# johncreed/one-class-ffm

Hardware: AMD Instinct MI355X
Metric: train instances/sec, kkbox-shape k=32; 1/2/4/8 MI355X vs CPU OpenMP (higher is better)
Workload: dtype f32; 1 GPU; kkbox-shape (BASELINE configs[2]): one-class FFM block Newton-CG epoch; rows_per_gpu=30755, rows_total=30755, items=100000, positives=2127663, user_fields=2, item_fields=3, k=32, parallelism=dp1, rccl_ranks=0, launcher=none, allreduce=none

## Files before the change

### one-class-ffm_amd/csrc/kernels.hpp

```cpp
#pragma once

#include <hip/hip_runtime.h>
#include <stdint.h>

#include <type_traits>

namespace ocffm {

typedef float f4v __attribute__((ext_vector_type(4)));
typedef double d2v __attribute__((ext_vector_type(2)));
typedef double d4v __attribute__((ext_vector_type(4)));

#ifndef OCFFM_F64_WIDE
#define OCFFM_F64_WIDE 1
#endif
template <typename real> struct VT;
template <> struct VT<float> {
  using V = f4v;
  static constexpr int N = 4;
};
template <> struct VT<double> {
  using V = std::conditional_t<OCFFM_F64_WIDE != 0, d4v, d2v>;
  static constexpr int N = OCFFM_F64_WIDE ? 4 : 2;
};
// ... 2572 lines not shown
                                                      const real *__restrict__ src, real *__restrict__ dst,
                                                      const int *__restrict__ skip) {
  if (skip && *skip) return;
  for (uint64_t q = ((uint64_t)blockIdx.x * BLOCK + threadIdx.x) * 4; q < n; q += (uint64_t)gridDim.x * BLOCK * 4) {
    if (q + 4 <= n) {
      const uint4 ix = *reinterpret_cast<const uint4 *>(idx + q);
      const real a = src[ix.x], b = src[ix.y], c = src[ix.z], d = src[ix.w];
      dst[q] = a;
      dst[q + 1] = b;
      dst[q + 2] = c;
      dst[q + 3] = d;
    } else {
      for (uint64_t r = q; r < n; r++) dst[r] = src[idx[r]];
    }
  }
}

template <typename real, int KP>
__global__ __launch_bounds__(BLOCK) void k_update_side_row(uint64_t R, const int64_t *__restrict__ xptr,
                                                           const uint32_t *__restrict__ xidx,
                                                           const real *__restrict__ xval, const real *__restrict__ S,
                                                           real *__restrict__ P1, const real *__restrict__ Q1,
                                                           real *__restrict__ a1, bool one, real *__restrict__ W,
                                                           const real *__restrict__ Pd, const CgState *st,
                                                           double *__restrict__ asum, double *part, unsigned *tick,
                                                           const int *__restrict__ skip, uint64_t nfold) {
  using G = Geo<real, KP>;
  if (skip && *skip) return;
  WAVE_SETUP
  const int sg = lane / G::LPR, li = lane % G::LPR;
  const real alpha = ((W || nfold) && st->nr_cg >= 1) ? (real)st->alpha : (real)0;
  double bs = 0;
  for (uint64_t i = wave * G::NSG + sg; i < R; i += nwaves * G::NSG) {
    vec_t<real> xs = vzero<real>();
    if (nfold) {
      for (int64_t p = one ? (int64_t)i : xptr[i]; p < (one ? (int64_t)i + 1 : xptr[i + 1]); p++)
        xs += vsplat<real>(xval[p]) * final_step<real>(S, Pd, alpha, (size_t)xidx[p] * KP + li * G::VE);
    } else if (W) {
      xs = vsplat<real>(xval[i]) * apply_owned_row<real, KP>(S, Pd, W, alpha, (size_t)xidx[i] * KP + li * G::VE);
    } else if (one) {
      xs = vsplat<real>(xval[i]) * vld<real>(S + (size_t)xidx[i] * KP + li * G::VE);
    } else {
      for (int64_t p = xptr[i]; p < xptr[i + 1]; p++)
        xs += vsplat<real>(xval[p]) * vld<real>(S + (size_t)xidx[p] * KP + li * G::VE);
    }
    vst<real>(P1 + i * KP + li * G::VE, vld<real>(P1 + i * KP + li * G::VE) + xs);
    const real gap = sg_sum<G::LPR>(hsum<real>(xs * vld<real>(Q1 + i * KP + li * G::VE)));
    if (li == 0) {
      const real an = a1[i] + gap;
      a1[i] = an;
      bs += (double)an;
    }
  }
  if (nfold) fold_apply<real>(nfold, S, Pd, W, alpha);
  const double bv[1] = {block_sum(bs)};
  double tot[1];
  if (last_block<1>(bv, part, tick, tot) && threadIdx.x == 0) asum[0] = tot[0];
}

template <typename real, int KP, int SPT>
__global__ __launch_bounds__(BLOCK) void k_gram_part(uint64_t Rp, int L, const real *const *__restrict__ A,
                                                     const real *__restrict__ B, const real *__restrict__ wv,
                                                     double *__restrict__ part, uint64_t rows_per_block,
                                                     int sub_per_y) {
  constexpr int Q4 = KP / 4;
  constexpr int TR = (KP >= 64) ? 16 : 32;
  constexpr int VE = VT<real>::N;
  extern __shared__ __align__(16) unsigned char smem_raw[];
  real *sA = reinterpret_cast<real *>(smem_raw);
  real *sB = sA + (size_t)L * TR * KP;
  real *sW = sB + (size_t)TR * KP;
  const int t = threadIdx.x;
  const int nsub_tot = L * Q4 * Q4;
  const int sub0 = blockIdx.y * sub_per_y;
  const int nsub = max(0, min(sub_per_y, nsub_tot - sub0));
  real acc[SPT][16];
#pragma unroll
  for (int q = 0; q < SPT; q++)
#pragma unroll
    for (int x = 0; x < 16; x++) acc[q][x] = 0;
  real cs = 0, ws = 0, wtot = 0;
  const uint64_t r0 = (uint64_t)blockIdx.x * rows_per_block;
  const uint64_t r1 = min(Rp, r0 + rows_per_block);
  const bool do_cols = blockIdx.y == 0;
  const int pieces_row = KP / VE;
  const int ntab = L + (B ? 1 : 0);
  for (uint64_t j0 = r0; j0 < r1; j0 += TR) {
    const int nr = (int)min<uint64_t>(TR, r1 - j0);
    __syncthreads();
    const int tot = ntab * TR * pieces_row;
    for (int q = t; q < tot; q += BLOCK) {
      const int tab = q / (TR * pieces_row);
      const int rr = (q / pieces_row) % TR;
      const int pc = q % pieces_row;
      vec_t<real> v = vzero<real>();
      if (rr < nr) v = vld<real>((tab < L ? A[tab] : B) + (j0 + rr) * KP + pc * VE);
      vst<real>((tab < L ? sA + ((size_t)tab * TR + rr) * KP : sB + (size_t)rr * KP) + pc * VE, v);
    }
    if (wv && t < TR) sW[t] = t < nr ? wv[j0 + t] : (real)0;
    __syncthreads();
#pragma unroll
    for (int q = 0; q < SPT; q++) {
      if (t + q * BLOCK < nsub) {
        const int sub = sub0 + t + q * BLOCK;
        const int l = sub / (Q4 * Q4), eq = (sub / Q4) % Q4, dq = sub % Q4;
        const real *pa = sA + (size_t)l * TR * KP + eq * 4;
        const real *pb = sB + dq * 4;
        for (int rr = 0; rr < nr; rr++) {
          real av[4], bv[4];
#pragma unroll
          for (int x = 0; x < 4; x++) {
            av[x] = pa[rr * KP + x];
            bv[x] = pb[rr * KP + x];
          }
#pragma unroll
          for (int x = 0; x < 4; x++)
#pragma unroll
            for (int y = 0; y < 4; y++) acc[q][x * 4 + y] += av[x] * bv[y];
        }
      }
    }
    if (do_cols && t < KP && B) {
      for (int rr = 0; rr < nr; rr++) {
        const real bb = sB[rr * KP + t];
        cs += bb;
        if (wv) ws += sW[rr] * bb;
      }
    }
    if (do_cols && t == 0 && wv)
      for (int rr = 0; rr < nr; rr++) wtot += sW[rr];
  }
  const size_t NOUT = (size_t)L * KP * KP + 2 * KP + 1;
  double *out = part + (size_t)blockIdx.x * NOUT;
#pragma unroll
  for (int q = 0; q < SPT; q++) {
    if (t + q * BLOCK < nsub) {
      const int sub = sub0 + t + q * BLOCK;
      const int l = sub / (Q4 * Q4), eq = (sub / Q4) % Q4, dq = sub % Q4;
#pragma unroll
      for (int x = 0; x < 4; x++)
#pragma unroll
        for (int y = 0; y < 4; y++) out[((size_t)l * KP + eq * 4 + x) * KP + dq * 4 + y] = (double)acc[q][x * 4 + y];
    }
  }
  if (do_cols) {
    if (t < KP) {
      out[(size_t)L * KP * KP + t] = (double)cs;
      out[(size_t)L * KP * KP + KP + t] = (double)ws;
    }
    if (t == 0) out[(size_t)L * KP * KP + 2 * KP] = (double)wtot;
  }
}

template <int L>
__global__ __launch_bounds__(BLOCK) void k_gram_mfma32(uint64_t Rp, const float *const *__restrict__ A,
                                                      const float *__restrict__ B, const float *__restrict__ wv,
                                                      float *__restrict__ part, uint64_t rows_per_block) {
  typedef float f16x __attribute__((ext_vector_type(16)));
  constexpr int U = 4;
  __shared__ float red[L][1024];
  __shared__ float redc[3][32];
  const int lane = threadIdx.x & 63, w = threadIdx.x >> 6;
  const int e = lane & 31, hf = lane >> 5;
  f16x acc[L];
#pragma unroll
  for (int c = 0; c < L; c++)
#pragma unroll
    for (int r = 0; r < 16; r++) acc[c][r] = 0.0f;
  BufView ab[L];
#pragma unroll
  for (int c = 0; c < L; c++) ab[c] = buf_view(A[c], Rp * 128);
  const BufView bb = buf_view(B, B ? Rp * 128 : 0), wb = buf_view(wv, wv ? Rp * 4 : 0);
  float cs = 0, ws = 0, wt = 0;
  const uint64_t r0 = (uint64_t)blockIdx.x * rows_per_block;
  const uint64_t r1 = min(Rp, r0 + rows_per_block);
  float bv[2][U], wvv[2][U], av[2][U][L];
  auto load = [&](int sb, uint64_t j0) {
#pragma unroll
    for (int u = 0; u < U; u++) {
      const uint64_t jj = j0 + 8 * u + hf;
      const bool ok = jj < r1;
      const uint32_t off = ok ? (uint32_t)(jj * 128 + e * 4) : 0xffffffffu;
      bv[sb][u] = bld1<float>(bb, off);
      wvv[sb][u] = bld1<float>(wb, ok ? (uint32_t)(jj * 4) : 0xffffffffu);
#pragma unroll
      for (int c = 0; c < L; c++) av[sb][u][c] = bld1<float>(ab[c], off);
    }
  };
  auto step = [&](int sb) {
#pragma unroll
    for (int u = 0; u < U; u++) {
#pragma unroll
      for (int c = 0; c < L; c++) acc[c] = __builtin_amdgcn_mfma_f32_32x32x2f32(av[sb][u][c], bv[sb][u], acc[c], 0, 0, 0);
      cs += bv[sb][u];
      ws += wvv[sb][u] * bv[sb][u];
      if (e == 0) wt += wvv[sb][u];
    }
  };
  for (uint64_t j0 = r0 + 2 * w; j0 < r1; j0 += 16 * U) {
    load(0, j0);
    load(1, j0 + 8 * U);
    step(0);
    step(1);
  }
  cs += __shfl_xor(cs, 32, 64);
  ws += __shfl_xor(ws, 32, 64);
  wt += __shfl_xor(wt, 32, 64);
  for (int ww = 0; ww < BLOCK / 64; ww++) {
    if (w == ww) {
#pragma unroll
      for (int c = 0; c < L; c++)
#pragma unroll
          for (int r = 0; r < 16; r++) {
            const int m = 8 * (r >> 2) + 4 * hf + (r & 3);
            float &x = red[c][m * 32 + e];
            x = (ww == 0 ? 0.0f : x) + acc[c][r];
          }
      if (hf == 0) {
        redc[0][e] = (ww == 0 ? 0.0f : redc[0][e]) + cs;
        redc[1][e] = (ww == 0 ? 0.0f : redc[1][e]) + ws;
        if (e == 0) redc[2][0] = (ww == 0 ? 0.0f : redc[2][0]) + wt;
      }
    }
    __syncthreads();
  }
  const size_t NOUT = (size_t)L * 1024 + 2 * 32 + 1;
  float *out = part + (size_t)blockIdx.x * NOUT;
  for (int o = threadIdx.x; o < L * 1024; o += BLOCK) out[o] = red[o >> 10][o & 1023];
  if (threadIdx.x < 32) {
    out[(size_t)L * 1024 + threadIdx.x] = redc[0][threadIdx.x];
    out[(size_t)L * 1024 + 32 + threadIdx.x] = redc[1][threadIdx.x];
  }
  if (threadIdx.x == 0) out[(size_t)L * 1024 + 64] = redc[2][0];
}

constexpr int GW64 = 1;
static __global__ __launch_bounds__(BLOCK, 3) void k_gram_mfma64(uint64_t Rp, int C, const float *const *__restrict__ A,
                                                       const float *__restrict__ B, const float *__restrict__ wv,
                                                       float *__restrict__ part, uint64_t nout,
                                                       uint64_t rows_per_block, unsigned ngroups, unsigned nwork) {
  typedef float f16x __attribute__((ext_vector_type(16)));
  constexpr int U = 4;
  const int lane = threadIdx.x & 63, w = threadIdx.x >> 6;
  const int e = lane & 31, hf = lane >> 5;
  const unsigned L = (gridDim.x & 7u) ? blockIdx.x : xcd_work_item(blockIdx.x, gridDim.x);
  if (L >= nwork) return;
  const unsigned grp = L % ngroups, chunk = L / ngroups;
  const int c0 = (int)(grp * (BLOCK / 64) + w);
  if (c0 > C) return;
  f16x acc[4];
#pragma unroll
  for (int t = 0; t < 4; t++)
#pragma unroll
    for (int r = 0; r < 16; r++) acc[t][r] = 0.0f;
  const BufView bb = buf_view(B, Rp * 256);
  const uint64_t r0 = (uint64_t)chunk * rows_per_block;
  const uint64_t r1 = r0 + rows_per_block < Rp ? r0 + rows_per_block : Rp;
  float *out = part + (size_t)chunk * nout;
  if (c0 == C) {
    const BufView wb = buf_view(wv, wv ? Rp * 4 : 0);
    float wt = 0;
    for (uint64_t j0 = r0; j0 < r1; j0 += 2 * U) {
      float bv[U][2], sv[U];
#pragma unroll
      for (int u = 0; u < U; u++) {
        const uint64_t jj = j0 + 2 * u + hf;
        const bool ok = jj < r1;
        const uint32_t off = ok ? (uint32_t)(jj * 256 + e * 4) : 0xffffff00u;
#pragma unroll
        for (int h = 0; h < 2; h++) bv[u][h] = bld1<float>(bb, off + h * 128);
        const float wvi = bld1<float>(wb, ok ? (uint32_t)(jj * 4) : 0xffffff00u);
        sv[u] = e == 0 ? 1.0f : (e == 1 ? wvi : 0.0f);
        if (e == 0) wt += wvi;
      }
#pragma unroll
      for (int u = 0; u < U; u++)
#pragma unroll
        for (int nt = 0; nt < 2; nt++) acc[nt] = __builtin_amdgcn_mfma_f32_32x32x2f32(sv[u], bv[u][nt], acc[nt], 0, 0, 0);
    }
    wt += __shfl_xor(wt, 32, 64);
    if (hf == 0) {
#pragma unroll
      for (int nt = 0; nt < 2; nt++) {
        out[(size_t)C * 4096 + nt * 32 + e] = acc[nt][0];
        out[(size_t)C * 4096 + 64 + nt * 32 + e] = acc[nt][1];
      }
      if (e == 0) out[(size_t)C * 4096 + 128] = wt;
    }
    return;
  }
  const BufView ab = buf_view(A[c0], Rp * 256);
  float bv[2][U][2], av[2][U][2];
  auto load = [&](int sb, uint64_t j0) {
#pragma unroll
    for (int u = 0; u < U; u++) {
      const uint64_t jj = j0 + 2 * u + hf;
      const uint32_t off = jj < r1 ? (uint32_t)(jj * 256 + e * 4) : 0xffffff00u;
#pragma unroll
      for (int h = 0; h < 2; h++) {
        bv[sb][u][h] = bld1<float>(bb, off + h * 128);
        av[sb][u][h] = bld1<float>(ab, off + h * 128);
      }
    }
  };
  auto step = [&](int sb) {
#pragma unroll
    for (int u = 0; u < U; u++)
#pragma unroll
      for (int mt = 0; mt < 2; mt++)
#pragma unroll
        for (int nt = 0; nt < 2; nt++)
          acc[mt * 2 + nt] = __builtin_amdgcn_mfma_f32_32x32x2f32(av[sb][u][mt], bv[sb][u][nt], acc[mt * 2 + nt], 0, 0, 0);
  };
  for (uint64_t j0 = r0; j0 < r1; j0 += 4 * U) {
    load(0, j0);
    load(1, j0 + 2 * U);
    step(0);
    step(1);
  }
#pragma unroll
  for (int t = 0; t < 4; t++)
#pragma unroll
    for (int r = 0; r < 16; r++) {
      const int m = (t >> 1) * 32 + 8 * (r >> 2) + 4 * hf + (r & 3), n = (t & 1) * 32 + e;
      out[(size_t)c0 * 4096 + m * 64 + n] = acc[t][r];
    }
}

static __global__ __launch_bounds__(BLOCK) void k_gram_mfma_f64(uint64_t Rp, int C, const double *const *__restrict__ A,
                                                               const double *__restrict__ B,
                                                               const double *__restrict__ wv, double *__restrict__ part,
                                                               uint64_t nout, uint64_t rows_per_block,
                                                               unsigned ngroups, unsigned nwork) {
  typedef double d4 __attribute__((ext_vector_type(4)));
  constexpr int U = 4;
  const int lane = threadIdx.x & 63, w = threadIdx.x >> 6;
  const int c16 = lane & 15, rq = lane >> 4;
  const unsigned L = (gridDim.x & 7u) ? blockIdx.x : xcd_work_item(blockIdx.x, gridDim.x);
  if (L >= nwork) return;
  const unsigned grp = L % ngroups, chunk = L / ngroups;
  const int c0 = (int)(grp * (BLOCK / 64) + w);
  if (c0 > C) return;
  const uint64_t r0 = (uint64_t)chunk * rows_per_block;
  const uint64_t r1 = r0 + rows_per_block < Rp ? r0 + rows_per_block : Rp;
  double *out = part + (size_t)chunk * nout;
  const BufView bb = buf_view(B, Rp * 256);
  if (c0 == C) {
    const BufView wb = buf_view(wv, wv ? Rp * 8 : 0);
    double cs[2] = {0, 0}, ws[2] = {0, 0}, wt = 0;
    for (uint64_t j0 = r0; j0 < r1; j0 += 4 * U) {
#pragma unroll
      for (int u = 0; u < U; u++) {
        const uint64_t jj = j0 + 4 * u + rq;
        const bool ok = jj < r1;
        const uint32_t off = ok ? (uint32_t)(jj * 256 + c16 * 8) : 0xffffff00u;
        const double wvi = bld1<double>(wb, ok ? (uint32_t)(jj * 8) : 0xffffff00u);
#pragma unroll
        for (int h = 0; h < 2; h++) {
          const double b = bld1<double>(bb, off + h * 128);
          cs[h] += b;
          ws[h] += wvi * b;
// ... 276 lines not shown
```

### one-class-ffm_amd/csrc/solver.hip

```cpp
#include <hip/hip_runtime.h>
#include <hip/hip_ext.h>
#include <rccl/rccl.h>

#include <algorithm>
#include <atomic>
#include <charconv>
#include <chrono>
#include <cmath>
#include <cstdio>
#include <cstdlib>
#include <cstring>
#include <fstream>
#include <iomanip>
#include <iostream>
#include <map>
#include <memory>
#include <stdexcept>
#include <string>
#include <thread>
#include <tuple>
#include <unordered_map>
#include <type_traits>
#include <vector>

// ... 1704 lines not shown
    }
    pending_.clear();
  }

  void utx(DevSide<real> &s, uint32_t fi, const real *A, real *out) {
    if (s.R == 0) return;
    DevField<real> &F = *s.F[fi];
    with_kp(kp_, [&](auto K) {
      constexpr int KP = decltype(K)::value;
      using Gm = Geo<real, KP>;
      prof_launch("utx", 0, [&] {
        launch(k_utx<real, KP>, grid_for(s.R, 4 * Gm::NSG), BLOCK, 0, s.R, F.xptr.p, F.xidx.p, F.xval.p, A, out);
      });
    });
  }

  void rowdot_add(uint64_t R, const real *P, const real *Q, real *acc) {
    if (R == 0) return;
    with_kp(kp_, [&](auto K) {
      constexpr int KP = decltype(K)::value;
      using Gm = Geo<real, KP>;
      launch(k_rowdot_add<real, KP>, grid_for(R, 4 * Gm::NSG), BLOCK, 0, R, P, Q, acc);
      HIPCHK(hipGetLastError());
    });
  }

  void bias_sums() {
    for (int sd = 0; sd < 2; sd++) {
      DevSide<real> &s = sd ? V_ : U_;
      launch(k_vec_sum<real>, grid_for(s.R, BLOCK, 256), BLOCK, 0, (uint64_t)s.R, (const real *)s.bias.p,
             bsum_.p + sd, part_.p, tick_.p);
    }
  }

  void calc_side() {
    for (uint32_t f1 = 0; f1 < f_; f1++)
      for (uint32_t f2 = f1; f2 < f_; f2++) {
        if ((f1 < fu_) != (f2 < fu_)) continue;
        const uint32_t b12 = block_index(f1, f2, f_);
        DevSide<real> &s = side(f1);
        rowdot_add(s.R, P_[b12].p, Q_[b12].p, s.bias.p);
      }
  }

  void init_y_tilde() {
    if (U_.R == 0) return;
    with_kp(kp_, [&](auto K) {
      constexpr int KP = decltype(K)::value;
      launch(k_init_ytilde<real, KP>, grid_for(U_.R, 4), BLOCK, 0,
          U_.R, U_.yptr.p, U_.ycol.p, U_.yt.p, V_.yt.p, U_.perm.p, (int)C_, (const real *const *)tabs_.p,
          (const real *const *)(tabs_.p + C_), U_.bias.p, V_.bias.p);
      HIPCHK(hipGetLastError());
    });
  }

  static constexpr int GRAM_LMAX = 8;
  bool mfma_gram(int L) const { return std::is_same<real, float>::value && kp_ == 32 && L >= 1 && !no_mfma_; }

  void aggregates(uint64_t Rp, int L, const real *const *A, const real *B, const real *wv, real *M) {
    const size_t rs = sizeof(real);
    if (mfma_gram64(L, Rp)) {
      gram64(Rp, L, A, B, wv, M);
      return;
    }
    if (std::is_same<real, double>::value && kp_ == 32 && L >= 1 && !no_mfma_ && B_ok(Rp) && M && B) {
      gram_f64(Rp, L, A, B, wv, M);
      return;
    }
    const int TR = kp_ >= 64 ? 16 : 32;
    const bool mg = mfma_gram(L) && (uint64_t)Rp * 128 < 0xffffff00ull;
    const int lmax = mg ? GRAM_LMAX
                                  : std::max<int>(1, (int)((64 * 1024 / rs - (size_t)TR * kp_ - TR) / ((size_t)TR * kp_)));
    int l0 = 0;
    bool first = true;
    do {
      const int Lc = std::min(L - l0, lmax);
      launch_aggr(Rp, Lc, A ? A + l0 : nullptr, B, first ? wv : nullptr, M ? M + (size_t)l0 * kp_ * kp_ : nullptr,
                  first, mg);
      l0 += Lc;
      first = false;
    } while (l0 < L);
  }

  bool mfma_gram64(int L, uint64_t Rp) const {
    return std::is_same<real, float>::value && kp_ == 64 && L >= 1 && !no_mfma_ && B_ok(Rp);
  }
  static bool B_ok(uint64_t Rp) { return Rp * 256 < 0xffffff00ull; }
  void gram64(uint64_t Rp, int L, const real *const *A, const real *B, const real *wv, real *M) {
    if (!M || !B) throw Error(OCFFM_E_STATE, "gram64: Grams and partner table required");
    constexpr int TPB = (BLOCK / 64) * GW64;
    const unsigned gy = (unsigned)((L + 1 + TPB - 1) / TPB);
    const uint64_t nout = (uint64_t)L * 4096 + 129;
    uint64_t nbx = std::max<uint64_t>(1, std::min<uint64_t>((Rp + 63) / 64, std::max<uint64_t>(1, gram64_blocks_ / gy)));
    const uint64_t rpb = ((Rp + nbx - 1) / nbx + 15) / 16 * 16;
    nbx = std::max<uint64_t>(1, (Rp + rpb - 1) / rpb);
    if (gpart64_.n < nbx * nout) gpart64_.alloc(nbx * nout, false);
    const double abytes = (double)Rp * ((L + (B ? 1 : 0)) * 64 + (wv ? 1 : 0)) * sizeof(real);
    const unsigned nwork = (unsigned)(nbx * gy);
    const unsigned grid = xcd_order_ ? (nwork + 7) / 8 * 8 : nwork;
    prof_launch("aggregates", abytes, [&] {
      launch(k_gram_mfma64, grid, BLOCK, 0, Rp, L, (const float *const *)A, (const float *)B,
             (const float *)wv, gpart64_.p, nout, rpb, gy, nwork);
    }, 2.0 * Rp * L * 64 * 64);
    const uint64_t ng = (uint64_t)L * 4096, cnt = ng + 129;
    prof_launch("aggr_reduce", (double)nbx * cnt * 4, [&] {
      launch(k_reduce_parts<real, float>, (unsigned)((cnt + 15) / 16), BLOCK, 0, nbx, nout, (uint64_t)0, cnt,
             (const float *)gpart64_.p, ng, M, sums_.p);
    });
  }

  void gram_f64(uint64_t Rp, int L, const real *const *A, const real *B, const real *wv, real *M) {
    constexpr int TPB = BLOCK / 64;
    const unsigned gy = (unsigned)((L + 1 + TPB - 1) / TPB);
    const uint64_t nout = (uint64_t)L * 1024 + 65;
    uint64_t nbx = std::max<uint64_t>(1, std::min<uint64_t>((Rp + 63) / 64, std::max<uint64_t>(1, gram64_blocks_ / gy)));
    const uint64_t rpb = ((Rp + nbx - 1) / nbx + 31) / 32 * 32;
    nbx = std::max<uint64_t>(1, (Rp + rpb - 1) / rpb);
    if (gpartd_.n < nbx * nout) gpartd_.alloc(nbx * nout, false);
    const double abytes = (double)Rp * ((L + 1) * 32 + (wv ? 1 : 0)) * sizeof(real);
    const unsigned nwork = (unsigned)(nbx * gy);
    const unsigned grid = xcd_order_ ? (nwork + 7) / 8 * 8 : nwork;
    prof_launch("aggregates", abytes, [&] {
      launch(k_gram_mfma_f64, grid, BLOCK, 0, Rp, L, (const double *const *)A, (const double *)B,
             (const double *)wv, gpartd_.p, nout, rpb, gy, nwork);
    }, 2.0 * Rp * L * 32 * 32);
    const uint64_t ng = (uint64_t)L * 1024, cnt = ng + 65;
    prof_launch("aggr_reduce", (double)nbx * cnt * 8, [&] {
      launch(k_reduce_parts<real, double>, (unsigned)((cnt + 15) / 16), BLOCK, 0, nbx, nout, (uint64_t)0, cnt,
             (const double *)gpartd_.p, ng, M, sums_.p);
    });
  }

  void launch_aggr(uint64_t Rp, int L, const real *const *A, const real *B, const real *wv, real *M, bool sums,
                   bool mg) {
    const int TR = kp_ >= 64 ? 16 : 32;
    const size_t smem = ((size_t)L * TR * kp_ + (size_t)TR * kp_ + TR) * sizeof(real);
    const uint64_t nout = (uint64_t)L * kp_ * kp_ + 2 * kp_ + 1;
    const int nsub = L * (kp_ / 4) * (kp_ / 4);
    with_kp(kp_, [&](auto K) {
      constexpr int KP = decltype(K)::value;
      constexpr int SPT = KP >= 64 ? 4 : 2;
      const int sub_per_y = SPT * BLOCK;
      const unsigned gy = (unsigned)std::max(1, (nsub + sub_per_y - 1) / sub_per_y);
      uint64_t nbx = std::max<uint64_t>(1, std::min<uint64_t>((Rp + 63) / 64, 512 / gy));
      nbx = std::min<uint64_t>(nbx, std::max<uint64_t>(1, part_.n / nout));
      const uint64_t rpb = (Rp + nbx - 1) / nbx;
      const double abytes = (double)Rp * ((L + (B ? 1 : 0)) * kp_ + (wv ? 1 : 0)) * sizeof(real);
      if (mg) {
        nbx = std::max<uint64_t>(1, std::min<uint64_t>((Rp + 127) / 128, gram_blocks_));
        nbx = std::min<uint64_t>(nbx, std::max<uint64_t>(1, part_.n / nout));
        const uint64_t rpbm = (Rp + nbx - 1) / nbx;
        prof_launch("aggregates", abytes, [&] {
          auto go = [&](auto lc) {
            launch(k_gram_mfma32<decltype(lc)::value>, (unsigned)nbx, BLOCK, 0, Rp, (const float *const *)A,
                   (const float *)B, (const float *)wv, (float *)part_.p, rpbm);
          };
          switch (L) {
            case 1: go(std::integral_constant<int, 1>()); break;
            case 2: go(std::integral_constant<int, 2>()); break;
            case 3: go(std::integral_constant<int, 3>()); break;
            case 4: go(std::integral_constant<int, 4>()); break;
            case 5: go(std::integral_constant<int, 5>()); break;
            case 6: go(std::integral_constant<int, 6>()); break;
            case 7: go(std::integral_constant<int, 7>()); break;
            default: go(std::integral_constant<int, GRAM_LMAX>()); break;
          }
        });
      } else {
        prof_launch("aggregates", abytes, [&] {
          launch(k_gram_part<real, KP, SPT>, dim3((unsigned)nbx, gy), BLOCK, smem, Rp, L, A, B, wv, part_.p,
                                                                                        rpb, sub_per_y);
        });
      }
      const uint64_t ng = (uint64_t)L * KP * KP;
      const uint64_t gm = M ? ng : 0, off = M ? 0 : ng, cnt = gm + (sums ? 2 * KP + 1 : 0);
      if (cnt)
        prof_launch("aggr_reduce", (double)nbx * cnt * (mg ? 4 : 8), [&] {
          if (mg)
            launch(k_reduce_parts<real, float>, (unsigned)((cnt + 15) / 16), BLOCK, 0, nbx, nout, off, cnt,
                   (const float *)part_.p, gm, M, sums_.p);
          else
            launch(k_reduce_parts<real>, (unsigned)((cnt + 15) / 16), BLOCK, 0, nbx, nout, off, cnt,
                   (const double *)part_.p, gm, M, sums_.p);
        });
      HIPCHK(hipGetLastError());
    });
  }

  void allreduce_dev(real *buf, uint64_t count) {
    if (!comm_.active()) return;
    if (comm_.nccl) {
      NCCLCHK(ncclAllReduce(buf, buf, count, std::is_same<real, double>::value ? ncclDouble : ncclFloat, ncclSum,
                            comm_.nccl, stream_));
    } else {
      HIPCHK(hipMemcpyAsync(stage_, buf, count * sizeof(real), hipMemcpyDeviceToHost, stream_));
      sync();
      if (comm_.host_fn(stage_, count, std::is_same<real, double>::value, comm_.host_user) != 0)
        throw Error(OCFFM_E_COMM, "host all-reduce callback failed");
      HIPCHK(hipMemcpyAsync(buf, stage_, count * sizeof(real), hipMemcpyHostToDevice, stream_));
    }
  }

  void allreduce_dev_d(double *buf, uint64_t count) {
    if (!comm_.active()) return;
    if (comm_.nccl) {
      NCCLCHK(ncclAllReduce(buf, buf, count, ncclDouble, ncclSum, comm_.nccl, stream_));
    } else {
      if (count > DSTAGE) throw Error(OCFFM_E_ARG, "allreduce_dev_d: too many values");
      HIPCHK(hipMemcpyAsync(dstage_, buf, count * sizeof(double), hipMemcpyDeviceToHost, stream_));
      sync();
      if (comm_.host_fn(dstage_, count, 1, comm_.host_user) != 0)
        throw Error(OCFFM_E_COMM, "host all-reduce callback failed");
      HIPCHK(hipMemcpyAsync(buf, dstage_, count * sizeof(double), hipMemcpyHostToDevice, stream_));
    }
  }

  void sync_owned() {
    if (!owned_stale_) return;
    owned_stale_ = false;
    for (uint32_t f1 = 0; f1 < f_; f1++)
      for (uint32_t f2 = f1; f2 < f_; f2++) {
        const uint32_t b12 = block_index(f1, f2, f_);
        if (!blocks_[b12].used) continue;
        for (int t = 0; t < 2; t++) {
          const uint32_t fl = t == 0 ? f1 : f2;
          DevField<real> &F = *side(fl).F[fidx(fl)];
          if (!F.excl) continue;
          real *T = t == 0 ? W_[b12].p : H_[b12].p;
          with_kp(kp_, [&](auto K) {
            constexpr int KP = decltype(K)::value;
            using Gm = Geo<real, KP>;
            const uint64_t nv = F.D * KP / Gm::VE;
            launch(k_mask_rows<real>, grid_for(nv, BLOCK, 2048), BLOCK, 0, nv, T, F.own.p, (uint32_t)Gm::LPR);
          });
          allreduce_dev(T, F.D * kp_);
        }
      }
    sync();
  }

  void allreduce_host(double *buf, uint64_t count) {
    if (!comm_.active()) return;
    if (comm_.nccl) {
      DevBuf<double> d;
      d.upload(buf, count);
      NCCLCHK(ncclAllReduce(d.p, d.p, count, ncclDouble, ncclSum, comm_.nccl, stream_));
      HIPCHK(hipMemcpyAsync(buf, d.p, count * sizeof(double), hipMemcpyDeviceToHost, stream_));
      sync();
    } else if (comm_.host_fn(buf, count, 1, comm_.host_user) != 0) {
      throw Error(OCFFM_E_COMM, "host all-reduce callback failed");
    }
  }

  const double *at_double(DevBuf<real> &at, uint64_t mt) {
    at_d_.alloc(std::max<uint64_t>(mt, 1));
    if (mt) {
      std::vector<real> t(mt);
      HIPCHK(hipMemcpyAsync(t.data(), at.p, mt * sizeof(real), hipMemcpyDeviceToHost, stream_));
      sync();
      std::vector<double> d(t.begin(), t.end());
      HIPCHK(hipMemcpy(at_d_.p, d.data(), mt * sizeof(double), hipMemcpyHostToDevice));
    }
    return at_d_.p;
  }

  struct HalfCtx {
    uint32_t b12, fl, fo;
    bool cross, user;
    DevSide<real> *own, *partner;
    DevField<real> *F;
    uint64_t D;
    real *W1, *P1, *Q1;
    const real *fw;
  };

  HalfCtx half_ctx(uint32_t f1, uint32_t f2, int which) {
    HalfCtx h;
    h.b12 = block_index(f1, f2, f_);
    if (!blocks_[h.b12].used) throw Error(OCFFM_E_ARG, "block not in the model (--ns)");
    h.fl = which == 0 ? f1 : f2;
    h.fo = which == 0 ? f2 : f1;
    h.user = h.fl < fu_;
    h.cross = (f1 < fu_) != (f2 < fu_);
    h.own = &side(h.fl);
    h.partner = h.cross ? &side(h.fo) : h.own;
    h.F = h.own->F[fidx(h.fl)].get();
    h.D = h.F->D;
    h.W1 = which == 0 ? W_[h.b12].p : H_[h.b12].p;
    h.P1 = which == 0 ? P_[h.b12].p : Q_[h.b12].p;
    h.Q1 = which == 0 ? Q_[h.b12].p : P_[h.b12].p;
    h.fw = prm_.freq ? h.F->freqw.p : nullptr;
    return h;
  }

  void gradient(HalfCtx &h) {
    DevSide<real> &own = *h.own;
    if (!(lazy_ok_ && h.cross)) flush_base();
    if (h.cross) ysum_dirty();
    with_kp(kp_, [&](auto K) {
      constexpr int KP = decltype(K)::value;
      using Gm = Geo<real, KP>;
      const double rs = sizeof(real);
      if (h.cross) {
        DevSide<real> &ps = *h.partner;
        aggregates(ps.R, (int)C_, partner_tabs(h), h.Q1, ps.bias.p, M_.p);
        const size_t msz = (size_t)C_ * KP * KP * sizeof(real);
        const bool lds = msz <= 64 * 1024;
        double bytes = (double)own.R * 8 + (double)own.npos * (4 + rs) + (double)ps.R * KP * rs +
// ... 1431 lines not shown
      if (e.tag > nr || (e.tag == -1 && !queued)) e.name += ".noop";
    }
    ccg_now_ = hot_now_ = false;
    cg_log.push_back(nr);
    account_half(h, nr);
    if (hb) {
      hipEvent_t he = ev();
      HIPCHK(hipEventRecord(he, stream_));
      char name[32];
      std::snprintf(name, sizeof(name), "half(%u,%u)%c", f1, f2, which ? 'H' : 'W');
      pending_.push_back({name, 0.0, hb, he, 0, 0.0});
    }
  }

  void finish_half(HalfCtx &h, const int *skip) {
    DevSide<real> &own = *h.own;
    if (h.cross) ysum_dirty();
    else ysum_ok_[h.user ? 1 : 0] = false;
    with_kp(kp_, [&](auto K) {
      constexpr int KP = decltype(K)::value;
      using Gm = Geo<real, KP>;
      const double rs = sizeof(real);
      const uint64_t nv = h.D * KP / Gm::VE;
      const bool excl = h.F->excl;
      if (excl) owned_stale_ = true;
      DevField<real> &F = *h.F;
      const bool fold = F.idlike && own.R > 0 && !excl && !no_fold_;
      const bool rows_kernel = !h.cross || (excl_.on && excl_.b12 == h.b12);
      const bool gfold = !fold && own.R > 0 && !excl && !no_fold_ && gfold_on_ && rows_kernel;
      real *Wf = (fold || gfold) ? h.W1 : nullptr;
      const uint64_t nfold = gfold ? nv : 0;
      const double fbytes = gfold ? (double)h.D * KP * rs * 4 : 0.0;
      if (!fold && !gfold)
        prof_launch("apply_step", (double)h.D * KP * rs * 5, [&] {
          launch(k_apply<real>, grid_for(nv, BLOCK, 2048), BLOCK, 0, nv, Vd_.p, S_.p, h.W1, st_.p,
                 excl ? (const uint8_t *)h.F->own.p : nullptr, (uint32_t)Gm::LPR, skip);
        });
      if (own.R == 0) return;
      if (h.cross) {
        DevSide<real> &other = *h.partner;
        if (excl_.on && excl_.b12 == h.b12) {
          prof_launch("update_cross_rows", (double)own.R * 16 + (double)F.nnz * (4 + rs) + (double)F.D * KP * rs +
                                               (double)own.R * KP * rs * 2 + fbytes, [&] {
            launch(k_update_cross_rows<real, KP>, mfill(k_update_cross_rows<real, KP>, grid_for(own.R, 4 * Gm::NSG)), BLOCK, 0, own.R, F.xptr.p, F.xidx.p,
                   F.xval.p, (const real *)S_.p, h.P1, (real *)nullptr, F.one, Wf, (const real *)Vd_.p,
                   (const CgState *)st_.p, skip, nfold);
          });
          return;
        }
        const double bytes = (double)own.R * 16 + (double)F.nnz * (4 + rs) + (double)F.D * KP * rs +
                             (double)own.R * KP * rs * 2 + (double)own.npos * (4 + 2 * rs) +
                             (double)other.R * KP * rs;
        prof_launch("update_cross_row", bytes, [&] {
          launch(k_update_cross_seg<real, KP>, mfill(k_update_cross_seg<real, KP>, grid_for(own.nseg, 4 * Gm::NSG)), BLOCK, 0,
              own.nseg, own.segs.p, F.xptr.p, F.xidx.p, F.xval.p, S_.p, h.P1, own.ycol.p, own.yt.p, h.Q1,
              (uint64_t)other.R, F.segd.p, F.segx.p, Wf,
              (const real *)Vd_.p, (const CgState *)st_.p, (const real *)nullptr, (const real *)nullptr,
              (const real *)nullptr, skip);
        });
        refresh_other(own, other, skip);
      } else {
        DevSide<real> &other = h.user ? V_ : U_;
        const double bytes = (double)own.R * 16 + (double)F.nnz * (4 + rs) + (double)F.D * KP * rs +
                             (double)own.R * KP * rs * 3 + (double)own.R * rs * 2 + (double)own.npos * (4 + 4 * rs) + fbytes;
        prof_launch("update_side_row", bytes, [&] {
          launch(k_update_side_row<real, KP>, mfill(k_update_side_row<real, KP>, grid_for(own.R, 4 * Gm::NSG)), BLOCK, 0,
              own.R, F.xptr.p, F.xidx.p, F.xval.p, S_.p, h.P1, h.Q1, own.bias.p, F.one, Wf,
              (const real *)Vd_.p, (const CgState *)st_.p, bsum_.p + (h.user ? 0 : 1), part_.p, tick_.p, skip, nfold);
        });
      }
    });
  }

  void account_half(const HalfCtx &h, int c) {
    const double s = sizeof(real), k = (double)kp_;
    const double R = (double)h.own->R, D = (double)h.D, P = (double)h.own->npos;
    const double csr = 8 * R + (double)h.F->nnz * (4 + s);
    if (!h.cross) {
      const double Rp = (double)(h.user ? V_.R : U_.R);
      const double gd = P * s + 8 * R + 2 * R * s + Rp * s + R * k * s + csr + 2 * D * k * s;
      const double hs = c * (8 * R + R * k * s + csr + 9 * D * k * s);
      const double upd = 4 * D * k * s + csr + 3 * R * k * s + 2 * R * s + 2 * P * s + 8 * R;
      alg_bytes += gd + hs + upd;
    } else {
      const double Rp = (double)h.partner->R, Cc = (double)C_;
      const double gd = (Cc + 2) * Rp * k * s + Rp * s + Cc * R * k * s + 8 * R + P * (4 + s) + R * s + csr +
                        2 * D * k * s;
      const double hs = Rp * k * s + c * (csr + 8 * R + 4 * P + Rp * k * s + 9 * D * k * s);
      const double upd = 4 * D * k * s + csr + 2 * R * k * s + 2 * P * s + 4 * P + 8 * R + Rp * k * s;
      alg_bytes += gd + hs + upd;
    }
  }

  ocffm_param prm_;
  Comm comm_;
  DevBuf<int64_t> gvptr_;
  double gn1_ = 0;
  bool has_test_;
  bool inited_ = false;
  hipStream_t stream_ = nullptr;
  uint32_t k_, kp_, fu_, fv_, f_, C_ = 0;
  double w_, lam_, r_;
  uint64_t m_glob_ = 0, n_ = 0, u0_ = 0, u1_ = 0, dmax_ = 0, npop_ = 0;
  uint64_t seg_len_ = std::is_same<real, double>::value ? 48 : 32;

  int lookahead_ = 1;
  bool spec_on_ = !std::getenv("OCFFM_SPEC") || std::atoi(std::getenv("OCFFM_SPEC")) != 0;
  std::vector<int> pred_;
  bool ysum_on_ = !std::getenv("OCFFM_YSUM") || std::atoi(std::getenv("OCFFM_YSUM")) != 0;
  bool exact_r2_ = std::getenv("OCFFM_EXACT_R2") && std::atoi(std::getenv("OCFFM_EXACT_R2")) != 0;
  bool ysum_ok_[2] = {false, false};
  DevBuf<real> yrow_;
  bool yrow_ok_[2] = {false, false};
  bool gfold_on_ = !std::getenv("OCFFM_GFOLD") || std::atoi(std::getenv("OCFFM_GFOLD")) != 0;
  bool ytvia_ = !std::getenv("OCFFM_YTVIA") || std::atoi(std::getenv("OCFFM_YTVIA")) != 0;
  bool side_refresh_ = std::getenv("OCFFM_SIDE_REFRESH") && std::atoi(std::getenv("OCFFM_SIDE_REFRESH")) != 0;
  hipStream_t side_ = nullptr;
  hipEvent_t side_ev_[2] = {nullptr, nullptr};
  bool side_pending_ = false;
  bool tpre_on_ = std::getenv("OCFFM_TPRE") && std::atoi(std::getenv("OCFFM_TPRE")) != 0;
  DevBuf<real> Tpre_;
  unsigned tpre_blocks_ = std::getenv("OCFFM_TPRE_BLOCKS") ? (unsigned)std::max(1, std::atoi(std::getenv("OCFFM_TPRE_BLOCKS"))) : 256;
  bool tpre(uint64_t R, uint64_t npos) const {
    const bool big = (size_t)C_ * kp_ * kp_ * sizeof(real) > 64 * 1024;
    const bool few = tpre_few_ && R >= 65536 && npos < 4 * R;
    return (tpre_on_ || big || few) && std::is_same<real, float>::value && (kp_ == 32 || kp_ == 64) && C_ >= 1 &&
           R > 0 && (uint64_t)R * kp_ * sizeof(real) < 0xffffff00ull && !no_mfma_;
  }
  bool tpre_few_ = !std::getenv("OCFFM_TPRE_FEW") || std::atoi(std::getenv("OCFFM_TPRE_FEW")) != 0;
  DevBuf<real> ysum_;
  void ysum_dirty() { ysum_ok_[0] = ysum_ok_[1] = false; }
  uint64_t hot_min_ = 0;
  DevBuf<real> hotG_, hotP_;
  int hot_steps_ = 6;
  bool hot_env_ = false;
  bool hot_now_ = false;
  int ccg_mode_ = std::getenv("OCFFM_CCG") ? std::atoi(std::getenv("OCFFM_CCG"))
                  : std::getenv("OCFFM_NO_MFMA") == nullptr ? 1 : 0;
  bool ccg_now_ = false;
  DevBuf<real> ccgG_, ccgP_;
  int spec_fixed_ = std::getenv("OCFFM_SPEC_FIXED") ? std::atoi(std::getenv("OCFFM_SPEC_FIXED")) : 0;
  bool fuse_ = true;
  bool coltau_on_ = !std::getenv("OCFFM_COLTAU") || std::atoi(std::getenv("OCFFM_COLTAU")) != 0;
  bool no_fold_ = std::getenv("OCFFM_NO_FOLD") != nullptr;
  int cgram_mode_ = std::getenv("OCFFM_CGRAM") ? std::atoi(std::getenv("OCFFM_CGRAM")) : 1;
  bool cgram_on_ = cgram_mode_ != 0;
  uint64_t cgram_chunk_ = std::getenv("OCFFM_CGRAM_CHUNK") ? std::max(1, std::atoi(std::getenv("OCFFM_CGRAM_CHUNK"))) : 128;
  bool no_mfma_ = std::getenv("OCFFM_NO_MFMA") != nullptr;
  DevBuf<float> gpart64_;
  DevBuf<double> gpartd_;
  bool tau_mfma_ = !std::getenv("OCFFM_TAU_MFMA") || std::atoi(std::getenv("OCFFM_TAU_MFMA")) != 0;
  bool xcd_order_ = !std::getenv("OCFFM_XCD_ORDER") || std::atoi(std::getenv("OCFFM_XCD_ORDER")) != 0;
  uint64_t gram64_blocks_ = std::getenv("OCFFM_GRAM64_BLOCKS") ? std::strtoull(std::getenv("OCFFM_GRAM64_BLOCKS"), nullptr, 10) : 1024;
  uint64_t gram_blocks_ = std::getenv("OCFFM_GRAM_BLOCKS") ? std::strtoull(std::getenv("OCFFM_GRAM_BLOCKS"), nullptr, 10) : 512;
  bool no_owned_ = false;
  bool host_build_ = std::getenv("OCFFM_HOST_BUILD") != nullptr && std::atoi(std::getenv("OCFFM_HOST_BUILD")) != 0;
  bool host_init_ = std::getenv("OCFFM_HOST_INIT") != nullptr && std::atoi(std::getenv("OCFFM_HOST_INIT")) != 0;
  bool owned_stale_ = false;
  unsigned hs_blocks_ = 4096;
  unsigned feat_blocks_ = 1024;
  hipEvent_t arm_a_ = nullptr, arm_b_ = nullptr;
  bool arm_first_ = false;
  DevSide<real> U_, V_, T_;
  unsigned rec_slices_ = 0;
  uint64_t rec_rows_ = 0;
  uint64_t rec_seg_ = 0;
  std::vector<Block> blocks_;
  std::vector<DevBuf<real>> W_, H_, P_, Q_;
  DevBuf<real> acc_, G_, S_, Vd_, Rv_, Hv_, h_, M_, wpart_;
  DevBuf<double> bsum_;
  struct ExclBase {
    bool on = false;
    uint32_t b12 = 0;
  } excl_;
  bool lazy_ok_ = false;
  bool lazy_base_ = !std::getenv("OCFFM_LAZY_BASE") || std::atoi(std::getenv("OCFFM_LAZY_BASE")) != 0;
  unsigned gd_blocks_ = std::getenv("OCFFM_GD_BLOCKS") ? (unsigned)std::atoi(std::getenv("OCFFM_GD_BLOCKS")) : 2048u;
  bool gd_fill_ = !std::getenv("OCFFM_GD_FILL") || std::atoi(std::getenv("OCFFM_GD_FILL")) != 0;
  bool feat_fill_ = !std::getenv("OCFFM_FEAT_FILL") || std::atoi(std::getenv("OCFFM_FEAT_FILL")) != 0;
  bool row_fill_ = std::getenv("OCFFM_ROW_FILL") ? std::atoi(std::getenv("OCFFM_ROW_FILL")) != 0
                                                 : std::is_same<real, float>::value;
  bool side_fill_ = !std::getenv("OCFFM_SIDE_FILL") || std::atoi(std::getenv("OCFFM_SIDE_FILL")) != 0;
  bool want_g_ = false;
  const real *qtq_ = nullptr;
  DevBuf<unsigned> tick_;
  DevBuf<double> sums_, vecs_, part_, at_d_, popular_;
  DevBuf<uint8_t> cold_;
  DevBuf<CgState> st_;
  DevBuf<real *> tabs_;
  int *run_host_ = nullptr, *run_host_dev_ = nullptr;
  DevBuf<unsigned> cgp_gen_buf_;
  DevBuf<int> cgp_abort_;
  unsigned cgp_gen_ = 1, ncu_ = 256;
  bool cgp_on_ = !std::getenv("OCFFM_CGP") || std::atoi(std::getenv("OCFFM_CGP")) != 0;
  bool cgp_xcd_ = !std::getenv("OCFFM_CGP_XCD") || std::atoi(std::getenv("OCFFM_CGP_XCD")) != 0;
  bool sidep_on_ = !std::getenv("OCFFM_SIDEP") || std::atoi(std::getenv("OCFFM_SIDEP")) != 0;
  bool sidef_on_ = !std::getenv("OCFFM_SIDE_FULL") || std::atoi(std::getenv("OCFFM_SIDE_FULL")) != 0;
  bool xfuse_on_ = !std::getenv("OCFFM_XFUSE") || std::atoi(std::getenv("OCFFM_XFUSE")) != 0;
  int xf_gb_ = std::getenv("OCFFM_XF_GB") ? std::atoi(std::getenv("OCFFM_XF_GB")) : (sizeof(real) == 8 ? 16 : 8);
  bool cgp_coop_ = std::getenv("OCFFM_CGP_COOP") && std::atoi(std::getenv("OCFFM_CGP_COOP")) != 0;
  unsigned cgp_spin_ = std::getenv("OCFFM_CGP_SPIN") ? (unsigned)std::atol(std::getenv("OCFFM_CGP_SPIN")) : CGP_SPIN_MAX;
  int cgp_stall_ = std::getenv("OCFFM_CGP_STALL") ? std::atoi(std::getenv("OCFFM_CGP_STALL")) : -1;
  real *stage_ = nullptr;
  static constexpr uint64_t DSTAGE = 64;
  double *dstage_ = nullptr;
  DevBuf<double> dots_;
  struct Pending {
    std::string name;
    double bytes;
    hipEvent_t a, b;
    int tag;
    double flops;
  };
  int prof_tag_ = 0;
  std::vector<Pending> pending_;
  std::vector<hipEvent_t> ev_pool_, ev_free_;
};

}

using namespace ocffm;

struct ocffm_problem {
  std::unique_ptr<ProblemBase> p;
};

extern "C" {

void ocffm_param_default(ocffm_param *p) {
  p->omega = 0.1;
  p->lambda = 1e-5;
  p->r = -1;
  p->nr_pass = 20;
  p->k = 4;
  p->nr_threads = 1;
  p->self_side = 1;
  p->freq = 0;
  p->precision = OCFFM_FP64;
  p->device = 0;
}

const char *ocffm_last_error(void) { return g_last_error.c_str(); }

int ocffm_device_count(int *count) {
  return guarded([&] {
    int c = 0;
    hipError_t e = hipGetDeviceCount(&c);
    *count = e == hipSuccess ? c : 0;
  });
}

int ocffm_data_read(const char *path, int has_label, const uint64_t *ds, uint32_t nds, ocffm_data **out) {
  return guarded([&] {
    auto d = std::make_unique<ocffm_data>();
    build(d->d, parse_rows(path, has_label != 0, ds, nds));
    d->d.path = path;
    *out = d.release();
  });
}

int ocffm_data_from_rows(uint64_t m, const uint64_t *xptr, const uint32_t *fid, const uint64_t *idx,
                         const double *val, const uint64_t *yptr, const uint64_t *ycol, const uint64_t *ds,
                         uint32_t nds, ocffm_data **out) {
  return guarded([&] {
    Rows r;
    r.has_label = yptr != nullptr;
    const uint64_t nn = xptr[m] - xptr[0];
    for (uint64_t p = xptr[0]; p < xptr[m]; p++) r.f = std::max<uint64_t>(r.f, (uint64_t)fid[p] + 1);
    if (ds == nullptr) {
      r.xptr.resize(m + 1);
      for (uint64_t i = 0; i <= m; i++) r.xptr[i] = xptr[i] - xptr[0];
      r.fid.assign(fid + xptr[0], fid + xptr[m]);
      r.idx.assign(idx + xptr[0], idx + xptr[m]);
      r.val.assign(val + xptr[0], val + xptr[m]);
    } else {
      r.fid.reserve(nn);
      r.idx.reserve(nn);
      r.val.reserve(nn);
      r.xptr.reserve(m + 1);
      for (uint64_t i = 0; i < m; i++) {
        for (uint64_t p = xptr[i]; p < xptr[i + 1]; p++) {
          if (fid[p] >= nds || ds[fid[p]] <= idx[p]) continue;
          r.fid.push_back(fid[p]);
          r.idx.push_back(idx[p]);
          r.val.push_back(val[p]);
        }
        r.xptr.push_back(r.fid.size());
      }
    }
    if (r.has_label) {
      r.yptr.resize(m + 1);
      for (uint64_t i = 0; i <= m; i++) r.yptr[i] = yptr[i] - yptr[0];
      r.ycol.assign(ycol + yptr[0], ycol + yptr[m]);
      for (uint64_t j : r.ycol) r.n = std::max<uint64_t>(r.n, j + 1);
    }
    auto d = std::make_unique<ocffm_data>();
    build(d->d, std::move(r));
    *out = d.release();
  });
}

int ocffm_data_trans_y(ocffm_data *V, const ocffm_data *U) {
  return guarded([&] { trans_y(V->d, U->d); });
}

int ocffm_data_get_info(const ocffm_data *d, ocffm_data_info *o) {
// ... 361 lines not shown
```

Measured before the change: 7.179 million instances/s.

## Software-pipeline the 32x32 MFMA gram kernel with a rotating triple buffer

Restructures the k_gram_mfma32 row loop into a rotating three-set register pipeline. Each step's MFMAs are followed right away by the load for the slot it just consumed, with sched_barriers keeping that order, so global loads overlap MFMA work instead of running load-all then compute-all. It also changes the row interleaving so each wave covers strided row pairs, makes the wave index wave-uniform, tightens buffer bounds to r1, and drops the lane-0 guard on wt. The cost is higher register pressure, which may reduce occupancy. An env flag can restore the old two-set schedule.

After: 7.207 million instances/s, median of 6. No clear change (+0.4%).

```diff
diff --git a/one-class-ffm_amd/csrc/kernels.hpp b/one-class-ffm_amd/csrc/kernels.hpp
--- a/one-class-ffm_amd/csrc/kernels.hpp
+++ b/one-class-ffm_amd/csrc/kernels.hpp
@@ -2748,61 +2748,93 @@
   }
 }
 
-template <int L>
+template <int L, bool ROT>
 __global__ __launch_bounds__(BLOCK) void k_gram_mfma32(uint64_t Rp, const float *const *__restrict__ A,
                                                       const float *__restrict__ B, const float *__restrict__ wv,
                                                       float *__restrict__ part, uint64_t rows_per_block) {
   typedef float f16x __attribute__((ext_vector_type(16)));
   constexpr int U = 4;
+  constexpr int NSET = ROT ? 3 : 2;
+  constexpr int NW = BLOCK / 64;
   __shared__ float red[L][1024];
   __shared__ float redc[3][32];
-  const int lane = threadIdx.x & 63, w = threadIdx.x >> 6;
+  const int lane = threadIdx.x & 63, w = __builtin_amdgcn_readfirstlane(threadIdx.x >> 6);
   const int e = lane & 31, hf = lane >> 5;
   f16x acc[L];
 #pragma unroll
   for (int c = 0; c < L; c++)
 #pragma unroll
     for (int r = 0; r < 16; r++) acc[c][r] = 0.0f;
-  BufView ab[L];
-#pragma unroll
-  for (int c = 0; c < L; c++) ab[c] = buf_view(A[c], Rp * 128);
-  const BufView bb = buf_view(B, B ? Rp * 128 : 0), wb = buf_view(wv, wv ? Rp * 4 : 0);
-  float cs = 0, ws = 0, wt = 0;
   const uint64_t r0 = (uint64_t)blockIdx.x * rows_per_block;
   const uint64_t r1 = min(Rp, r0 + rows_per_block);
-  float bv[2][U], wvv[2][U], av[2][U][L];
-  auto load = [&](int sb, uint64_t j0) {
-#pragma unroll
-    for (int u = 0; u < U; u++) {
-      const uint64_t jj = j0 + 8 * u + hf;
-      const bool ok = jj < r1;
-      const uint32_t off = ok ? (uint32_t)(jj * 128 + e * 4) : 0xffffffffu;
-      bv[sb][u] = bld1<float>(bb, off);
-      wvv[sb][u] = bld1<float>(wb, ok ? (uint32_t)(jj * 4) : 0xffffffffu);
-#pragma unroll
-      for (int c = 0; c < L; c++) av[sb][u][c] = bld1<float>(ab[c], off);
-    }
+  BufView ab[L];
+#pragma unroll
+  for (int c = 0; c < L; c++) ab[c] = buf_view(A[c], r1 * 128);
+  const BufView bb = buf_view(B, B ? r1 * 128 : 0), wb = buf_view(wv, wv ? r1 * 4 : 0);
+  float cs = 0, ws = 0, wt = 0;
+  float bv[NSET][U], wvv[NSET][U], av[NSET][U][L];
+  auto load1 = [&](int sb, int u, uint64_t j0) {
+    const uint64_t jj = j0 + 2 * NW * u;
+    const bool ok = jj < r1;
+    const uint32_t off = ok ? (uint32_t)(jj * 128) + lane * 4 : 0xffffffffu;
+    bv[sb][u] = bld1<float>(bb, off);
+    wvv[sb][u] = bld1<float>(wb, ok ? (uint32_t)(jj * 4) + hf * 4 : 0xffffffffu);
+#pragma unroll
+    for (int c = 0; c < L; c++) av[sb][u][c] = bld1<float>(ab[c], off);
   };
-  auto step = [&](int sb) {
-#pragma unroll
-    for (int u = 0; u < U; u++) {
-#pragma unroll
-      for (int c = 0; c < L; c++) acc[c] = __builtin_amdgcn_mfma_f32_32x32x2f32(av[sb][u][c], bv[sb][u], acc[c], 0, 0, 0);
-      cs += bv[sb][u];
-      ws += wvv[sb][u] * bv[sb][u];
-      if (e == 0) wt += wvv[sb][u];
-    }
+  auto step1 = [&](int sb, int u) {
+#pragma unroll
+    for (int c = 0; c < L; c++) acc[c] = __builtin_amdgcn_mfma_f32_32x32x2f32(av[sb][u][c], bv[sb][u], acc[c], 0, 0, 0);
+    cs += bv[sb][u];
+    float wb1 = wvv[sb][u] * bv[sb][u];
+    asm volatile("" : "+v"(wb1));
+    ws += wb1;
+    wt += wvv[sb][u];
+    asm volatile("" : "+v"(cs), "+v"(ws), "+v"(wt));
   };
-  for (uint64_t j0 = r0 + 2 * w; j0 < r1; j0 += 16 * U) {
-    load(0, j0);
-    load(1, j0 + 8 * U);
-    step(0);
-    step(1);
+  constexpr uint64_t S = 2 * NW * U;
+  const uint64_t jw = r0 + 2 * w;
+  if constexpr (ROT) {
+    const uint64_t ns = jw < r1 ? (r1 - jw + S - 1) / S : 0;
+#pragma unroll
+    for (int sb = 0; sb < NSET; sb++)
+#pragma unroll
+      for (int u = 0; u < U; u++) load1(sb, u, jw + sb * S);
+    uint64_t j0 = jw + NSET * S;
+    for (uint64_t p = ns / NSET; p; p--, j0 += NSET * S) {
+#pragma unroll
+      for (int sb = 0; sb < NSET; sb++)
+#pragma unroll
+        for (int u = 0; u < U; u++) {
+          step1(sb, u);
+          __builtin_amdgcn_sched_barrier(0);
+          load1(sb, u, j0 + sb * S);
+          __builtin_amdgcn_sched_barrier(0);
+        }
+    }
+    const unsigned tail = (unsigned)(ns % NSET);
+#pragma unroll
+    for (int sb = 0; sb + 1 < NSET; sb++)
+      if (sb < (int)tail) {
+#pragma unroll
+        for (int u = 0; u < U; u++) step1(sb, u);
+      }
+  } else {
+    for (uint64_t j0 = jw; j0 < r1; j0 += 2 * S) {
+#pragma unroll
+      for (int sb = 0; sb < 2; sb++)
+#pragma unroll
+        for (int u = 0; u < U; u++) load1(sb, u, j0 + sb * S);
+#pragma unroll
+      for (int sb = 0; sb < 2; sb++)
+#pragma unroll
+        for (int u = 0; u < U; u++) step1(sb, u);
+    }
   }
   cs += __shfl_xor(cs, 32, 64);
   ws += __shfl_xor(ws, 32, 64);
   wt += __shfl_xor(wt, 32, 64);
-  for (int ww = 0; ww < BLOCK / 64; ww++) {
+  for (int ww = 0; ww < NW; ww++) {
     if (w == ww) {
 #pragma unroll
       for (int c = 0; c < L; c++)
diff --git a/one-class-ffm_amd/csrc/solver.hip b/one-class-ffm_amd/csrc/solver.hip
--- a/one-class-ffm_amd/csrc/solver.hip
+++ b/one-class-ffm_amd/csrc/solver.hip
@@ -1880,8 +1880,13 @@
         const uint64_t rpbm = (Rp + nbx - 1) / nbx;
         prof_launch("aggregates", abytes, [&] {
           auto go = [&](auto lc) {
-            launch(k_gram_mfma32<decltype(lc)::value>, (unsigned)nbx, BLOCK, 0, Rp, (const float *const *)A,
-                   (const float *)B, (const float *)wv, (float *)part_.p, rpbm);
+            constexpr int LC = decltype(lc)::value;
+            if (gram_rot_)
+              launch(k_gram_mfma32<LC, true>, (unsigned)nbx, BLOCK, 0, Rp, (const float *const *)A,
+                     (const float *)B, (const float *)wv, (float *)part_.p, rpbm);
+            else
+              launch(k_gram_mfma32<LC, false>, (unsigned)nbx, BLOCK, 0, Rp, (const float *const *)A,
+                     (const float *)B, (const float *)wv, (float *)part_.p, rpbm);
           };
           switch (L) {
             case 1: go(std::integral_constant<int, 1>()); break;
@@ -3619,6 +3624,7 @@
   bool tau_mfma_ = !std::getenv("OCFFM_TAU_MFMA") || std::atoi(std::getenv("OCFFM_TAU_MFMA")) != 0;
   bool xcd_order_ = !std::getenv("OCFFM_XCD_ORDER") || std::atoi(std::getenv("OCFFM_XCD_ORDER")) != 0;
   uint64_t gram64_blocks_ = std::getenv("OCFFM_GRAM64_BLOCKS") ? std::strtoull(std::getenv("OCFFM_GRAM64_BLOCKS"), nullptr, 10) : 1024;
+  bool gram_rot_ = !std::getenv("OCFFM_GRAM_ROT") || std::atoi(std::getenv("OCFFM_GRAM_ROT")) != 0;
   uint64_t gram_blocks_ = std::getenv("OCFFM_GRAM_BLOCKS") ? std::strtoull(std::getenv("OCFFM_GRAM_BLOCKS"), nullptr, 10) : 512;
   bool no_owned_ = false;
   bool host_build_ = std::getenv("OCFFM_HOST_BUILD") != nullptr && std::atoi(std::getenv("OCFFM_HOST_BUILD")) != 0;
```
